# ZhangYuef/Alink

Measured on AMD Instinct MI355X. Metric: rows/sec/node + iters-to-converge, KMeans k=100 1e8-row×128-dim at 1/2/4/8 MI355X, higher is better.
Workload: dtype bf16

## Files before the change

### alink_amd/ops/_lib.py

```python
from __future__ import annotations

import ctypes
import os
from typing import Optional

import torch

__all__ = ["lib", "require", "available", "kernels_enabled", "call", "query", "LIB_PATH", "stream_ptr"]

LIB_PATH = os.environ.get("ALINK_HIP_LIB") or os.path.join(os.path.dirname(os.path.abspath(__file__)), "libalink_hip.so")
_lib: Optional[ctypes.CDLL] = None
_err: Optional[str] = None


def _load():
    global _lib, _err
    if _lib is not None or _err is not None:
        return _lib
    if not os.path.exists(LIB_PATH):
        _err = f"{LIB_PATH} not built (run python build_native.py)"
        return None
    try:
        L = ctypes.CDLL(LIB_PATH)
    except OSError as e:
# ... 19 lines not shown
    _lib = L
    return _lib


_c_i64, _c_int, _c_vp, _c_f = ctypes.c_int64, ctypes.c_int, ctypes.c_void_p, ctypes.c_float
_c_d = ctypes.c_double
_SIGNATURES = {
    "alink_kmeans_prep_centroids": [_c_vp, _c_int, _c_vp, _c_vp, _c_vp],
    "alink_kmeans_reduce_slabs": [_c_vp, _c_vp, _c_int, _c_int, _c_vp, _c_vp, _c_vp],
    "alink_tree_gather_rows": [_c_vp, _c_vp, _c_vp, _c_i64, _c_vp, _c_vp, _c_vp],
    "alink_tree_hist_fm": [_c_vp, _c_int, _c_vp, _c_vp, _c_vp, _c_int, _c_vp, _c_int, _c_int, _c_int, _c_vp, _c_int,
                           _c_int, _c_vp, _c_vp, _c_vp, _c_vp, _c_int],
    "alink_tree_hist_f32": [_c_vp, _c_i64, _c_int, _c_vp, _c_vp, _c_int, _c_int, _c_int, _c_vp, _c_int, _c_int,
                            _c_vp],
    "alink_tree_node_sums": [_c_vp, _c_vp, _c_vp, _c_i64, _c_int, _c_int, _c_vp, _c_int, _c_vp],
    "alink_tree_route": [_c_vp, _c_i64, _c_int, _c_vp, _c_vp, _c_vp, _c_vp, _c_int, _c_int, _c_vp],
    "alink_kmeans_assign_accum_bf16_v7": [_c_vp, _c_i64, _c_vp, _c_vp, _c_int, _c_vp, _c_vp, _c_int, _c_vp, _c_vp,
                                          _c_int],
    "alink_kmeans_v7_grid": [_c_i64, _c_int],
    "alink_kmeans_assign_accum_bf16_v10": [_c_vp, _c_i64, _c_vp, _c_vp, _c_int, _c_vp, _c_vp, _c_int, _c_vp, _c_vp,
                                           _c_int, _c_vp, _c_vp, _c_int, _c_d],
    "alink_kmeans_v10_grid": [_c_i64, _c_int],
    "alink_tree_predict": [_c_vp, _c_i64, _c_int, _c_int, _c_vp, _c_vp, _c_int, _c_vp, _c_vp, _c_int, _c_vp, _c_int,
                           _c_vp, _c_vp, _c_vp, _c_vp],
    "alink_tree_codes": [_c_vp, _c_int, _c_vp, _c_vp, _c_int, _c_i64, _c_i64, _c_int, _c_int, _c_vp, _c_vp],
    "alink_gbdt_rank_stats": [_c_vp, _c_vp, _c_vp, _c_vp, _c_int, _c_vp, _c_int, _c_vp, _c_vp, _c_vp, _c_vp],
    "alink_kmeans_seed_ref": [_c_vp, _c_vp, _c_vp, _c_int, _c_int, _c_int, _c_d, _c_vp, _c_vp, _c_vp, _c_vp],
    "alink_kmeans_local_lloyd": [_c_vp, _c_vp, _c_int, _c_int, _c_int, _c_vp, _c_vp, _c_vp, _c_vp, _c_vp, _c_int, _c_vp,
                                 _c_vp, _c_vp, _c_vp, _c_vp],
    "alink_kmeans_par_pick": [_c_vp, _c_i64, _c_i64, _c_i64, _c_d, _c_vp, _c_i64, _c_vp, _c_vp],
    "alink_kmeans_cost1_bf16": [_c_vp, _c_i64, _c_int, _c_vp, _c_vp, _c_vp, _c_int, _c_int, _c_vp],
    "alink_kmeans_nearest_bf16": [_c_vp, _c_i64, _c_int, _c_vp, _c_vp, _c_int, _c_int, _c_vp, _c_vp, _c_int,
                                  _c_int, _c_int, _c_vp, _c_vp],
    "alink_linear_grad_f64": [_c_vp, _c_vp, _c_vp, _c_vp, _c_i64, _c_int, _c_int, _c_d, _c_vp, _c_int, _c_vp,
                              _c_vp],
    "alink_linear_grad_pad": [_c_int],
    "alink_linear_search_f64": [_c_vp, _c_vp, _c_vp, _c_vp, _c_vp, _c_i64, _c_int, _c_int, _c_d, _c_d, _c_int, _c_vp,
                                _c_int, _c_vp, _c_vp],
    "alink_kmeans_update": [_c_vp, _c_int, _c_vp, _c_vp, _c_vp, _c_vp, _c_vp, _c_int, _c_vp, _c_d, _c_vp,
                            ctypes.c_uint64, _c_vp],
    "alink_kmeans_host_stat_alloc": [ctypes.POINTER(_c_vp), ctypes.POINTER(_c_vp)],
    "alink_kmeans_host_stat_free": [_c_vp],
    "alink_kmeans_accum_bf16": [_c_vp, _c_i64, _c_int, _c_vp, _c_vp, _c_int, _c_int, _c_vp, _c_vp, _c_vp, _c_vp],
    "alink_kmeans_accum_f32": [_c_vp, _c_i64, _c_int, _c_vp, _c_vp, _c_int, _c_int, _c_vp, _c_vp, _c_vp, _c_vp],
    "alink_kmeans_accum_kmax": [_c_int],
    "alink_kmeans_accum_mfma_bf16": [_c_vp, _c_i64, _c_vp, _c_int, _c_int, _c_vp, _c_vp, _c_vp, _c_vp],
    "alink_linear_grad_wide_f64": [_c_vp, _c_vp, _c_vp, _c_vp, _c_i64, _c_int, _c_int, _c_d, _c_vp, _c_int, _c_vp,
                                   _c_vp],
    "alink_csr_row_deriv_f64": [_c_vp, _c_vp, _c_vp, _c_vp, _c_vp, _c_vp, _c_i64, _c_int, _c_d, _c_vp, _c_vp, _c_vp],
    "alink_csc_gather_f64": [_c_vp, _c_vp, _c_vp, _c_vp, _c_i64, _c_vp, _c_vp],
    "alink_ftrl_check_indices": [_c_vp, _c_i64, _c_i64, _c_vp, _c_int, _c_vp],
    "alink_ftrl_hogwild_f64": [_c_vp, _c_vp, _c_vp, _c_vp, _c_i64, _c_vp, _c_vp, _c_vp, _c_d, _c_d, _c_d, _c_d, _c_int,
                               _c_vp],
    "alink_ftrl_partial_margin_f64": [_c_vp, _c_vp, _c_vp, _c_i64, _c_vp, _c_i64, _c_i64, _c_vp, _c_int, _c_vp],
    "alink_ftrl_coord_update_f64": [_c_vp, _c_i64, _c_vp, _c_vp, _c_vp, _c_vp, _c_vp, _c_vp, _c_i64, _c_i64, _c_d, _c_d,
                                    _c_d, _c_d, _c_i64, _c_int, _c_vp],
    "alink_ftrl_coord_scan_f64": [_c_vp, _c_vp, _c_vp, _c_i64, _c_vp, _c_vp, _c_vp, _c_vp, _c_vp, _c_i64, _c_d, _c_d,
                                  _c_d, _c_d, _c_int, _c_vp],
    "alink_ftrl_coord_long_f64": [_c_vp, _c_vp, _c_vp, _c_i64, _c_vp, _c_vp, _c_vp, _c_vp, _c_vp, _c_i64, _c_d, _c_d,
                                  _c_d, _c_d, _c_int, _c_vp],
    "alink_ftrl_prox_f64": [_c_vp, _c_i64, _c_vp, _c_vp, _c_vp, _c_d, _c_d, _c_d, _c_d, _c_int, _c_vp],
    "alink_murmur3_utf8_index": [_c_vp, _c_vp, _c_i64, _c_vp, _c_int, ctypes.c_uint32, _c_i64, _c_vp, _c_vp, _c_vp],
    "alink_murmur3_multi_index": [_c_vp, _c_int, _c_i64, ctypes.c_uint32, _c_i64, _c_vp, _c_vp, _c_vp],
    "alink_murmur3_bytes": [_c_vp, _c_vp, _c_i64, ctypes.c_uint32, _c_vp, _c_vp],
    "alink_vector_assemble": [_c_i64, _c_int, _c_vp, _c_vp, _c_vp, _c_vp, _c_int, _c_vp],
    "alink_murmur3_index": [_c_vp, _c_vp, _c_i64, _c_vp, _c_int, ctypes.c_uint32, _c_i64, _c_vp, _c_vp, _c_vp],
# ... 122 lines not shown
```

### alink_amd/ops/csrc/kmeans_v10.hip

```cpp
#include <hip/hip_runtime.h>
#include <stdint.h>
#include <stdlib.h>

#ifndef KM10_PAIRMAX
#define KM10_PAIRMAX 0
#endif

#ifndef KM10_TIMING
#define KM10_TIMING 0
#endif

#ifndef KM10_PFD
#define KM10_PFD 0
#endif

#include "kmeans_tile.h"
#include "kmeans_v10_body.h"

namespace {

using namespace kmtile;

typedef float f32x32 __attribute__((ext_vector_type(32)));
typedef float f32x16 __attribute__((ext_vector_type(16)));
typedef float f32x4v __attribute__((ext_vector_type(4)));
typedef uint32_t u32x4 __attribute__((ext_vector_type(4)));

enum Mode10 { FULL = 0, LOAD_ONLY = 1, COMPUTE_ONLY = 2, DIST_ONLY = 3, ACC_ONLY = 4 };

constexpr int NBUF = 9;
constexpr int AHEAD = 7;
constexpr int OFF_ASG = NBUF * TILE;
constexpr uint32_t IDX_MODE = 0xC000u;
constexpr int OFF_CNT = OFF_ASG + 512;
constexpr int OFF_DYN = OFF_CNT + 128 * 4;
constexpr int OFF_JUNK = OFF_DYN + 8 * 4;
constexpr int LDS_BYTES = OFF_JUNK + 256;
constexpr int CH = 16;
constexpr int RED_STRIDE = 112 * D;
static_assert(LDS_BYTES <= LDS_CAP && 2 * RED_STRIDE * 4 <= NBUF * TILE, "LDS plan");

__device__ __forceinline__ float pack(float v, uint32_t field) {
    return __uint_as_float((__float_as_uint(v) & 0xFFFFFF80u) | field);
}

__device__ __forceinline__ float max3_raw(float a, float b, float c) {
    float r;
    asm("v_max3_f32 %0, %1, %2, %3" : "=v"(r) : "v"(a), "v"(b), "v"(c));
    return r;
}
__device__ __forceinline__ float max_raw(float a, float b) {
    float r;
    asm("v_max_f32 %0, %1, %2" : "=v"(r) : "v"(a), "v"(b));
    return r;
}

template <int NT>
__device__ __forceinline__ void dma_tile(uint32_t m0v, uint32_t voff, __amdgpu_buffer_rsrc_t rs, uint32_t soff) {
    uint32_t keep, m1, s1, s2, s3;
#define KM10_DMA(POL)                                                                                       \
    asm volatile(                                                                                           \
        "s_mov_b32 %0, m0\n\t"                                                                              \
        "s_mov_b32 m0, %7\n\t"                                                                              \
        "s_add_u32 %2, %8, 4096\n\t"                                                                        \
        "buffer_load_dwordx4 %5, %6, %8 offen " POL " lds\n\t"                                              \
        "s_add_u32 %1, %7, 4096\n\t"                                                                        \
        "s_mov_b32 m0, %1\n\t"                                                                              \
        "s_add_u32 %3, %8, 8192\n\t"                                                                        \
        "buffer_load_dwordx4 %5, %6, %2 offen " POL " lds\n\t"                                              \
        "s_add_u32 %1, %7, 8192\n\t"                                                                        \
        "s_mov_b32 m0, %1\n\t"                                                                              \
        "s_add_u32 %4, %8, 12288\n\t"                                                                       \
        "buffer_load_dwordx4 %5, %6, %3 offen " POL " lds\n\t"                                              \
        "s_add_u32 %1, %7, 12288\n\t"                                                                       \
        "s_mov_b32 m0, %1\n\t"                                                                              \
        "s_nop 0\n\t"                                                                                       \
        "buffer_load_dwordx4 %5, %6, %4 offen " POL " lds\n\t"                                              \
        "s_mov_b32 m0, %0"                                                                                  \
        : "=&s"(keep), "=&s"(m1), "=&s"(s1), "=&s"(s2), "=&s"(s3)                                           \
        : "v"(voff), "s"(rs), "s"(m0v), "s"(soff)                                                           \
        : "memory")
    if constexpr (NT) KM10_DMA("nt");
    else KM10_DMA("");
#undef KM10_DMA
}

__device__ __forceinline__ void l2_touch(uint32_t m0v, uint32_t voff, __amdgpu_buffer_rsrc_t rs, uint32_t soff) {
    uint32_t keep;
    asm volatile(
        "s_mov_b32 %0, m0\n\t"
        "s_mov_b32 m0, %3\n\t"
        "s_nop 0\n\t"
        "buffer_load_dword %1, %2, %4 offen lds\n\t"
        "s_mov_b32 m0, %0"
        : "=&s"(keep)
        : "v"(voff), "s"(rs), "s"(m0v), "s"(soff)
        : "memory");
}

template <int KB, int MODE, int NT, int DYN>
__global__ __launch_bounds__(512) void kmeans_v10_kernel(const __bf16* __restrict__ Xp, int64_t N,
                                                         const __bf16* __restrict__ Cp,
                                                         const float* __restrict__ ninit, float* __restrict__ slab,
                                                         float* __restrict__ slab_cnt, int* __restrict__ assign_out,
                                                         int64_t ntiles, int64_t per, int rev,
                                                         unsigned* __restrict__ dyn_ctr, int dyn_par, int nqs,
                                                         int64_t pool_base, int npool,
                                                         const unsigned* __restrict__ skip, int pfd_arg) {
    static_assert(KB >= 1 && KB <= 7, "v10 holds at most 112 centroids in registers");
    const int pfd = KM10_PFD ? pfd_arg : 0;
    constexpr bool LOADS = MODE == FULL || MODE == LOAD_ONLY;
    __shared__ __attribute__((aligned(1024))) char lds[LDS_BYTES];
    if (skip != nullptr && __hip_atomic_load(skip, __ATOMIC_RELAXED, __HIP_MEMORY_SCOPE_AGENT) != 0u) return;
    const int tid = threadIdx.x;
    const int lane = tid & 63;
    const int wave = __builtin_amdgcn_readfirstlane(tid >> 6);
    const int g = lane >> 4;
// ... 144 lines not shown
        if (LOADS && dma_wave) {
            if (2 * j + AHEAD - 2 < ntp) stage_tile(2 * j + AHEAD - 2);
            if (2 * j + AHEAD - 1 < ntp) stage_tile(2 * j + AHEAD - 1);
        }
    };

    if (wave < 4) {
        const int myrow = 16 * wave + li;
        const int apos = 16 * ((myrow >> 2) & 3) + 4 * (myrow >> 4) + (myrow & 3);
        bf16x8 cf[KB][4];
        f32x4 nin[KB];
#pragma unroll
        for (int b = 0; b < KB; ++b) {
#pragma unroll
            for (int s = 0; s < 4; ++s)
                cf[b][s] = *reinterpret_cast<const bf16x8*>(Cp + (16 * b + li) * D + 8 * (s + 4 * g));
            nin[b] = *reinterpret_cast<const f32x4*>(ninit + 16 * b + 4 * g);
        }
        int xr[4];
#pragma unroll
        for (int s = 0; s < 4; ++s) xr[s] = xoff(myrow, s + 4 * g);
        auto load_frag = [&](uint32_t slot, bf16x8 (&x)[4]) {
            const char* xt = lds + slot;
#pragma unroll
            for (int s = 0; s < 4; ++s) x[s] = *reinterpret_cast<const bf16x8*>(xt + xr[s]);
        };
        auto cross_max = [&](float run) {
            const uint32_t u = __float_as_uint(run);
            const auto p32 = __builtin_amdgcn_permlane32_swap(u, u, false, false);
            const uint32_t u2 = __float_as_uint(max_raw(__uint_as_float(p32[0]), __uint_as_float(p32[1])));
            const auto p16 = __builtin_amdgcn_permlane16_swap(u2, u2, false, false);
            return __float_as_uint(max_raw(__uint_as_float(p16[0]), __uint_as_float(p16[1])));
        };
        auto rare_neg = [&](const bf16x8 (&x)[4], uint32_t u, uint32_t c) {
            float run = -3.4e38f;
#pragma unroll
            for (int b = 0; b < KB; ++b) {
                f32x4 acc = nin[b];
#pragma unroll
                for (int s = 0; s < 4; ++s) acc = __builtin_amdgcn_mfma_f32_16x16x32_bf16(cf[b][s], x[s], acc, 0, 0, 0);
                const uint32_t c0 = (uint32_t)(16 * b + 4 * g);
                run = max3_raw(run, pack(acc[0], c0), pack(acc[1], c0 + 1));
                run = max3_raw(run, pack(acc[2], c0 + 2), pack(acc[3], c0 + 3));
            }
            const uint32_t v = cross_max(run);
            return (int32_t)u < 0 ? (v & 127u) : c;
        };
        auto tile_max = [&](const bf16x8 (&x)[4]) {
            f32x4 acc[KB];
            float run = -3.4e38f;
#pragma unroll
            for (int b = 0; b <= KB + 1; ++b) {
                if (b < KB) {
                    acc[b] = nin[b];
#pragma unroll
                    for (int s = 0; s < 4; ++s)
                        acc[b] = __builtin_amdgcn_mfma_f32_16x16x32_bf16(cf[b][s], x[s], acc[b], 0, 0, 0);
                }
                if (b >= 2) {
                    const uint32_t f0 = 127u - (uint32_t)(16 * (b - 2) + 4 * g);
                    run = max3_raw(run, pack(acc[b - 2][0], f0), pack(acc[b - 2][1], f0 - 1));
                    run = max3_raw(run, pack(acc[b - 2][2], f0 - 2), pack(acc[b - 2][3], f0 - 3));
                }
                if (b < KB && b >= 2) {
#pragma unroll
                    for (int s = 0; s < 3; ++s) {
                        __builtin_amdgcn_sched_group_barrier(0x008, 1, 0);
                        __builtin_amdgcn_sched_group_barrier(0x002, 2, 0);
                    }
                    __builtin_amdgcn_sched_group_barrier(0x008, 1, 0);
                }
                __builtin_amdgcn_sched_barrier(0);
            }
            const uint32_t u = cross_max(run);
            uint32_t c = 127u - (u & 127u);
            if (__builtin_amdgcn_ballot_w64((int32_t)u < 0) != 0) c = rare_neg(x, u, c);
            return c;
        };
        auto pair_max = [&](const bf16x8 (&xa_)[4], const bf16x8 (&xb_)[4], uint32_t& ca, uint32_t& cb) {
            f32x4 aA[KB], aB[KB];
            float runA = -3.4e38f, runB = -3.4e38f;
#pragma unroll
            for (int b = 0; b <= KB + 1; ++b) {
                if (b < KB) {
                    aA[b] = nin[b];
                    aB[b] = nin[b];
#pragma unroll
                    for (int s = 0; s < 4; ++s) {
                        aA[b] = __builtin_amdgcn_mfma_f32_16x16x32_bf16(cf[b][s], xa_[s], aA[b], 0, 0, 0);
                        aB[b] = __builtin_amdgcn_mfma_f32_16x16x32_bf16(cf[b][s], xb_[s], aB[b], 0, 0, 0);
                    }
                }
                if (b >= 2) {
                    const uint32_t f0 = 127u - (uint32_t)(16 * (b - 2) + 4 * g);
                    runA = max3_raw(runA, pack(aA[b - 2][0], f0), pack(aA[b - 2][1], f0 - 1));
                    runA = max3_raw(runA, pack(aA[b - 2][2], f0 - 2), pack(aA[b - 2][3], f0 - 3));
                    runB = max3_raw(runB, pack(aB[b - 2][0], f0), pack(aB[b - 2][1], f0 - 1));
                    runB = max3_raw(runB, pack(aB[b - 2][2], f0 - 2), pack(aB[b - 2][3], f0 - 3));
                }
                if (b < KB && b >= 2) {
#pragma unroll
                    for (int s = 0; s < 6; ++s) {
                        __builtin_amdgcn_sched_group_barrier(0x008, 1, 0);
                        __builtin_amdgcn_sched_group_barrier(0x002, 2, 0);
                    }
                    __builtin_amdgcn_sched_group_barrier(0x008, 2, 0);
                }
                __builtin_amdgcn_sched_barrier(0);
            }
            const uint32_t uA = cross_max(runA), uB = cross_max(runB);
            ca = 127u - (uA & 127u);
            cb = 127u - (uB & 127u);
            if (__builtin_amdgcn_ballot_w64((int32_t)(uA | uB) < 0) != 0) {
                ca = rare_neg(xa_, uA, ca);
                cb = rare_neg(xb_, uB, cb);
            }
        };
        const int64_t row_end = DYN ? N : ((tbase + nt) * TR < N ? (tbase + nt) * TR : N);
        auto publish = [&](int j, int h, uint32_t c) {
            if (g == 0) {
                const int64_t grow = (DYN ? dphys(2 * j + h) : tbase + phys(2 * j + h)) * TR + myrow;
                reinterpret_cast<uint16_t*>(lds + OFF_ASG)[(j & 1) * 128 + h * 64 + apos] =
                    (uint16_t)(IDX_MODE | (2 * c));
                if (grow < row_end) {
                    __hip_atomic_fetch_add(cnt + c, 1u, __ATOMIC_RELAXED, __HIP_MEMORY_SCOPE_WORKGROUP);
                    if (assign_out != nullptr) assign_out[grow] = (int)c;
                }
            }
        };
        bf16x8 xa[4], xb[4];
        int pend = 0;
        unsigned pend_v = 0u;
        uint32_t slot_a = 0;
#if KM10_TIMING
        const uint64_t loop0 = __builtin_readcyclecounter();
#endif
        for (int j = 0; DYN || j <= np; ++j) {
            pre(j);
            if constexpr (DYN) {
                if (j > np_dyn) break;
                if (wave == 0) {
                    int nq = dstate[2 * (j & 1)], done = dstate[2 * (j & 1) + 1];
                    if (pend) {
                        const unsigned r = __builtin_amdgcn_readfirstlane(pend_v);
                        if ((int)r < npool) {
                            if (lane == 0)
                                qbase[nq & 3] = (int)(pool_base + (int64_t)(rev ? npool - 1 - (int)r : (int)r) * CH);
                            ++nq;
                        } else {
                            done = 1;
                        }
                        pend = 0;
                    }
                    if (!done && nq <= (2 * j + 2 * AHEAD - 4) / CH) {
                        if (lane == 0)
                            pend_v = __hip_atomic_fetch_add(dyn_ctr + dyn_par, 1u, __ATOMIC_RELAXED,
                                                            __HIP_MEMORY_SCOPE_AGENT);
                        pend = 1;
                    }
                    if (lane == 0) {
                        dstate[2 * ((j + 1) & 1)] = nq;
                        dstate[2 * ((j + 1) & 1) + 1] = done;
                    }
                }
            }
            const int npj = DYN ? np_dyn : np;
            if (MODE == LOAD_ONLY || MODE == ACC_ONLY || j >= npj) continue;
            const uint32_t slot_b = next_slot(slot_a);
            load_frag(slot_a, xa);
            load_frag(slot_b, xb);
            slot_a = next_slot(slot_b);
            uint32_t c0, c1;
            if constexpr (KM10_PAIRMAX) {
                pair_max(xa, xb, c0, c1);
            } else {
                c0 = tile_max(xa);
                c1 = tile_max(xb);
            }
            publish(j, 0, c0);
            publish(j, 1, c1);
#if KM10_TIMING
            if (j == 0 && tid == 0) stamp[1] = (int64_t)__builtin_amdgcn_s_memrealtime();
#endif
        }
#if KM10_TIMING
        if (tid == 0) {
            stamp[2] = (int64_t)__builtin_amdgcn_s_memrealtime();
            stamp[8] = (int64_t)wait_vm_cyc;
            stamp[9] = (int64_t)wait_bar_cyc;
            stamp[10] = (int64_t)(__builtin_readcyclecounter() - loop0);
        }
#endif
        barrier_lds();
        barrier_lds();
        barrier_lds();
    } else {
        const int a = wave - 4;
        const uint32_t aoff =
            lbase + (uint32_t)(a * 1024) + ((uint32_t)(16 * (lane >> 2) + 4 * (lane & 3)) ^ (uint32_t)(a << 4));
        f32x32 s0 = {}, s1 = {}, s2 = {}, s3 = {}, s4 = {}, s5 = {}, s6 = {};
        f32x16 xv = {};
        auto acc_tile = [&](uint32_t slot, const u32x4& v0, const u32x4& v1) {
            const uint32_t w0 = __builtin_amdgcn_readfirstlane(v0[0]), w1 = __builtin_amdgcn_readfirstlane(v0[1]);
            const uint32_t w2 = __builtin_amdgcn_readfirstlane(v0[2]), w3 = __builtin_amdgcn_readfirstlane(v0[3]);
            const uint32_t w4 = __builtin_amdgcn_readfirstlane(v1[0]), w5 = __builtin_amdgcn_readfirstlane(v1[1]);
            const uint32_t w6 = __builtin_amdgcn_readfirstlane(v1[2]), w7 = __builtin_amdgcn_readfirstlane(v1[3]);
            const uint32_t base = aoff + slot;
            f32x4v addr;
            uint32_t keep;
            asm volatile(KM10_ACC_BODY
                         : "+{v[32:63]}"(s0), "+{v[64:95]}"(s1), "+{v[96:127]}"(s2), "+{v[128:159]}"(s3),
// ... 190 lines not shown
```

### alink_amd/ops/kmeans.py

```python
from __future__ import annotations

import os
import weakref
from typing import Dict, Optional, Tuple

import numpy as np
import torch

from . import _lib
from . import kmeans_dense64 as _d64

__all__ = ["assign_accumulate", "assign", "assign_accumulate_torch", "hip_supported", "prepare_centroids",
           "general_supported", "assign_accumulate_general_hip", "accumulate_by_index_hip", "f32_supported",
           "assign_accumulate_f32_hip", "assign_f32"]

_BUF: Dict[Tuple, Tuple[torch.Tensor, torch.Tensor]] = {}
HIP_CALLS = 0
HIP_D = 128
HIP_KMAX = 128


def hip_supported(X: torch.Tensor, k: int) -> bool:
    return (X.is_cuda and X.dtype == torch.bfloat16 and X.dim() == 2 and X.shape[1] == HIP_D
            and 1 <= k <= HIP_KMAX and X.shape[0] > 0 and X.is_contiguous() and X.data_ptr() % 16 == 0)
# ... 297 lines not shown

def cost1_hip(X: torch.Tensor, c: torch.Tensor, with_sum: bool = False):
    if not nearest_supported(X):
        raise ValueError("cost1_hip needs contiguous bf16 [N, D] on GPU with D in (64, 128, 256)")
    n, d = X.shape
    cb = c.reshape(-1).to(device=X.device, dtype=torch.bfloat16).contiguous()
    if cb.numel() != d:
        raise ValueError("center shape mismatch")
    cost = torch.empty(n, dtype=torch.float64, device=X.device)
    grid = COST1_GRID * _num_cus(X.device)
    wsum = torch.empty(grid * 4, dtype=torch.float64, device=X.device) if with_sum else None
    _lib.call("alink_kmeans_cost1_bf16", X.data_ptr(), n, d, cb.data_ptr(), cost.data_ptr(),
              None if wsum is None else wsum.data_ptr(), grid, COST1_VARIANT, _lib.stream_ptr(X.device))
    return (cost, wsum) if with_sum else cost


def nearest_counts_hip(X: torch.Tensor, C: torch.Tensor) -> torch.Tensor:
    if not nearest_supported(X):
        raise ValueError("nearest_counts_hip needs contiguous bf16 [N, D] on GPU with D in (64, 128, 256)")
    n, d = X.shape
    m = C.shape[0]
    if m > NEAREST_CHUNK:
        return torch.bincount(nearest_hip(X, C)[0].to(torch.int64), minlength=m)
    Cb = C.to(device=X.device, dtype=torch.bfloat16).contiguous()
    if Cb.shape[1] != d or m == 0:
        raise ValueError("centroid shape mismatch")
    chalf = (0.5 * (Cb.float() ** 2).sum(1)).contiguous()
    counts = torch.zeros(m, dtype=torch.int64, device=X.device)
    _lib.call("alink_kmeans_nearest_bf16", X.data_ptr(), n, d, Cb.data_ptr(), chalf.data_ptr(), m, 0, None, None, 0,
              NEAREST_GRID * _num_cus(X.device), _rg(d, m), counts.data_ptr(), _lib.stream_ptr(X.device))
    return counts


def _scores(Xc: torch.Tensor, C: torch.Tensor, emulate_bf16: bool) -> torch.Tensor:
    if emulate_bf16:
        cb = C.to(torch.bfloat16).float()
        return Xc.float() @ cb.T - 0.5 * (cb ** 2).sum(1)
    Cd = C.to(Xc.dtype)
    return Xc @ Cd.T - 0.5 * (Cd ** 2).sum(1)


def assign_accumulate_torch(X: torch.Tensor, C: torch.Tensor, weights: Optional[torch.Tensor] = None,
                            chunk: int = 1 << 20) -> torch.Tensor:
    k, d = C.shape
    out = torch.zeros((k, d + 1), dtype=torch.float64, device=X.device)
    low = X.dtype in (torch.bfloat16, torch.float16)
    for s in range(0, X.shape[0], chunk):
        xc = X[s:s + chunk]
        if not low:
            xc = xc.to(torch.float64)
        idx = _scores(xc, C, low).argmax(1)
        w = None if weights is None else weights[s:s + chunk].to(torch.float64)
        xs = xc.to(torch.float64)
        if w is not None:
            xs = xs * w[:, None]
        out[:, :d].index_add_(0, idx, xs)
        out[:, d].index_add_(0, idx, torch.ones_like(idx, dtype=torch.float64) if w is None else w)
    return out


def general_supported(X: torch.Tensor, k: int) -> bool:
    return nearest_supported(X) and 1 <= k <= (512 if X.shape[1] == 64 else 256)


GENERAL_CALLS = 0
_ACC: Dict[Tuple, Tuple[torch.Tensor, torch.Tensor]] = {}
# ... 271 lines not shown
```

### alink_amd/ops/kmeans_rows.py

```python
from __future__ import annotations

from typing import Optional

import torch

from . import _lib, bisecting as bops, kmeans as kops, kmeans_dense64 as kd64, kmeans_sparse as ksp
from .kmeans_sparse import sparse_selected

__all__ = ["rows", "Rows", "column_kind", "sparse_selected", "sparse_rows", "pairwise_distance"]

CHUNK = 1 << 20
SPARSE_CHUNK = 1 << 16
SPARSE, DENSE, UNDECIDED = 1, 0, -1


def pairwise_distance(X: torch.Tensor, C: torch.Tensor, distance_type: str) -> torch.Tensor:
    dt = distance_type.upper()
    if dt == "COSINE":
        return 1.0 - X @ C.T
    if dt == "HAVERSINE":
        lat1 = torch.deg2rad(X[:, 0:1])
        lon1 = torch.deg2rad(X[:, 1:2])
        lat2 = torch.deg2rad(C[:, 0])[None, :]
        lon2 = torch.deg2rad(C[:, 1])[None, :]
# ... 189 lines not shown
    def _descend(self, table, slot, levels, grid):
        return _torch_descend(lambda M: self.X @ M.T, table, slot, levels)

    def _child_stats(self, slot, nslots, sqnorm, grid, work=None):
        from .gemm import tn_matmul
        X, d = self.X, self.d
        ok = (slot >= 0) & (slot < nslots)
        Xs, ps = X[ok], slot[ok].to(torch.int64)
        norm2 = self.row_sqnorm()[ok]
        onehot = torch.nn.functional.one_hot(ps, nslots).to(X.dtype)
        return torch.zeros((nslots, d + 2), dtype=torch.float64, device=X.device) + tn_matmul(
            onehot, torch.cat([Xs, torch.ones_like(norm2)[:, None], norm2[:, None]], 1))

    def queue_assign(self, k):
        if not kops.hip_supported(self.X, k):
            return None
        return lambda C, step, skip: kops.assign_accumulate_hip(self.X, C, reverse=kops.serpentine_reverse(step),
                                                                skip=skip)


class _Bf16Rows(_TorchRows):

    def nearest(self, C, dist_all=None):
        if C.shape[0] == 1:
            return torch.zeros(1, dtype=torch.int64, device=self.device).expand(self.n), kops.cost1_hip(self.X, C[0])
        idx, d2 = kops.nearest_hip(self.X, C)
        return idx.to(torch.int64), d2.to(torch.float64).sqrt_()

    def first_cost(self, c):
        cost, psum = kops.cost1_hip(self.X, c[0], with_sum=True)
        return cost, psum.sum()

    def nearest_counts(self, C):
        return kops.nearest_counts_hip(self.X, C)


class _Dense64Rows(_TorchRows):

    def nearest(self, C, dist_all=None):
        if dist_all is not None:
            return super().nearest(C, dist_all)
        idx, d2 = kd64.nearest(self.X, C, self.dist_type)
        return idx, (d2.sqrt_() if self.dist_type == "EUCLIDEAN" else d2)

    def nearest_counts(self, C):
        return kd64.nearest_counts(self.X, C, self.dist_type)

    def _descend(self, table, slot, levels, grid):
        if kd64.use_hip(self.X, 1):
            return bops.descend_f64(self.X, table, slot, levels, grid)
        return super()._descend(table, slot, levels, grid)

    def _child_stats(self, slot, nslots, sqnorm, grid, work=None):
        if not kd64.use_hip(self.X, nslots):
            return super()._child_stats(slot, nslots, sqnorm, grid)
        X, d = self.X, self.d
        if work is None:
            work = kd64.sorted_work(slot, nslots, ignore_outside=True)
        buf = torch.zeros((nslots, d + 2), dtype=torch.float64, device=X.device)
        buf[:, :d + 1] = kd64.accumulate_work(X, work, nslots, grid)
        if sqnorm:
            buf[:, d + 1] = kd64.accumulate_work(self.row_sqnorm()[:, None], work, nslots, grid)[:, 0]
        return buf


def rows(X, dist_type: str) -> Rows:
# ... 15 lines not shown
```

Measured before the change: 23.54 billion.

## Add ring-buffered MFMA kernel for k-means candidate weight counting

Adds a dedicated HIP kernel that counts nearest-candidate assignments for up to 224 bf16 candidates of 128 dims. It reuses the v10 LDS ring-DMA staging (shared helpers are moved into a header) and splits the candidate blocks across two wave groups, merging partial argmax results through LDS. Counts are accumulated with LDS atomics per workgroup. The bf16 rows path now uses this kernel for nearest_counts when the input is large enough. This is meant to replace the generic nearest kernel in the k-means|| weighting step. It adds a second specialized kernel to maintain, and the two-half merge is new logic whose tie-breaking may differ slightly from the old path.

```diff
diff --git a/alink_amd/ops/_lib.py b/alink_amd/ops/_lib.py
--- a/alink_amd/ops/_lib.py
+++ b/alink_amd/ops/_lib.py
@@ -75,6 +75,7 @@
     "alink_kmeans_cost1_bf16": [_c_vp, _c_i64, _c_int, _c_vp, _c_vp, _c_vp, _c_int, _c_int, _c_vp],
     "alink_kmeans_nearest_bf16": [_c_vp, _c_i64, _c_int, _c_vp, _c_vp, _c_int, _c_int, _c_vp, _c_vp, _c_int,
                                   _c_int, _c_int, _c_vp, _c_vp],
+    "alink_kmeans_weights_bf16_ring": [_c_vp, _c_i64, _c_vp, _c_int, _c_vp, _c_int, _c_int, _c_vp],
     "alink_linear_grad_f64": [_c_vp, _c_vp, _c_vp, _c_vp, _c_i64, _c_int, _c_int, _c_d, _c_vp, _c_int, _c_vp,
                               _c_vp],
     "alink_linear_grad_pad": [_c_int],
diff --git a/alink_amd/ops/csrc/kmeans_ring.h b/alink_amd/ops/csrc/kmeans_ring.h
--- /dev/null
+++ b/alink_amd/ops/csrc/kmeans_ring.h
@@ -0,0 +1,66 @@
+#pragma once
+#include "kmeans_tile.h"
+
+namespace kmring {
+
+using namespace kmtile;
+
+constexpr int NBUF = 9;
+constexpr int AHEAD = 7;
+
+__device__ __forceinline__ float max3_raw(float a, float b, float c) {
+    float r;
+    asm("v_max3_f32 %0, %1, %2, %3" : "=v"(r) : "v"(a), "v"(b), "v"(c));
+    return r;
+}
+__device__ __forceinline__ float max_raw(float a, float b) {
+    float r;
+    asm("v_max_f32 %0, %1, %2" : "=v"(r) : "v"(a), "v"(b));
+    return r;
+}
+
+template <int NT>
+__device__ __forceinline__ void dma_tile(uint32_t m0v, uint32_t voff, __amdgpu_buffer_rsrc_t rs, uint32_t soff) {
+    uint32_t keep, m1, s1, s2, s3;
+#define KM10_DMA(POL)                                                                                       \
+    asm volatile(                                                                                           \
+        "s_mov_b32 %0, m0\n\t"                                                                              \
+        "s_mov_b32 m0, %7\n\t"                                                                              \
+        "s_add_u32 %2, %8, 4096\n\t"                                                                        \
+        "buffer_load_dwordx4 %5, %6, %8 offen " POL " lds\n\t"                                              \
+        "s_add_u32 %1, %7, 4096\n\t"                                                                        \
+        "s_mov_b32 m0, %1\n\t"                                                                              \
+        "s_add_u32 %3, %8, 8192\n\t"                                                                        \
+        "buffer_load_dwordx4 %5, %6, %2 offen " POL " lds\n\t"                                              \
+        "s_add_u32 %1, %7, 8192\n\t"                                                                        \
+        "s_mov_b32 m0, %1\n\t"                                                                              \
+        "s_add_u32 %4, %8, 12288\n\t"                                                                       \
+        "buffer_load_dwordx4 %5, %6, %3 offen " POL " lds\n\t"                                              \
+        "s_add_u32 %1, %7, 12288\n\t"                                                                       \
+        "s_mov_b32 m0, %1\n\t"                                                                              \
+        "s_nop 0\n\t"                                                                                       \
+        "buffer_load_dwordx4 %5, %6, %4 offen " POL " lds\n\t"                                              \
+        "s_mov_b32 m0, %0"                                                                                  \
+        : "=&s"(keep), "=&s"(m1), "=&s"(s1), "=&s"(s2), "=&s"(s3)                                           \
+        : "v"(voff), "s"(rs), "s"(m0v), "s"(soff)                                                           \
+        : "memory")
+    if constexpr (NT) KM10_DMA("nt");
+    else KM10_DMA("");
+#undef KM10_DMA
+}
+
+__device__ __forceinline__ uint32_t ring_next_slot(uint32_t s) {
+    return s == (uint32_t)((NBUF - 1) * TILE) ? 0u : s + (uint32_t)TILE;
+}
+
+__device__ __forceinline__ uint32_t ring_lane_offset(int tid) {
+    const int prow = (tid & 255) >> 4;
+    return (uint32_t)(prow * ROWB + ((tid & 15) ^ xsw(prow)) * 16);
+}
+
+__device__ __forceinline__ void ring_wait_pair(int j, int ntp) {
+    const int issued = 2 * j + AHEAD - 3 < ntp - 1 ? 2 * j + AHEAD - 3 : ntp - 1;
+    wait_tile_np<4, 3>(issued - (2 * j + 1));
+}
+
+}
diff --git a/alink_amd/ops/csrc/kmeans_v10.hip b/alink_amd/ops/csrc/kmeans_v10.hip
--- a/alink_amd/ops/csrc/kmeans_v10.hip
+++ b/alink_amd/ops/csrc/kmeans_v10.hip
@@ -15,11 +15,13 @@
 #endif
 
 #include "kmeans_tile.h"
+#include "kmeans_ring.h"
 #include "kmeans_v10_body.h"
 
 namespace {
 
 using namespace kmtile;
+using namespace kmring;
 
 typedef float f32x32 __attribute__((ext_vector_type(32)));
 typedef float f32x16 __attribute__((ext_vector_type(16)));
@@ -28,8 +30,6 @@
 
 enum Mode10 { FULL = 0, LOAD_ONLY = 1, COMPUTE_ONLY = 2, DIST_ONLY = 3, ACC_ONLY = 4 };
 
-constexpr int NBUF = 9;
-constexpr int AHEAD = 7;
 constexpr int OFF_ASG = NBUF * TILE;
 constexpr uint32_t IDX_MODE = 0xC000u;
 constexpr int OFF_CNT = OFF_ASG + 512;
@@ -42,47 +42,6 @@
 
 __device__ __forceinline__ float pack(float v, uint32_t field) {
     return __uint_as_float((__float_as_uint(v) & 0xFFFFFF80u) | field);
-}
-
-__device__ __forceinline__ float max3_raw(float a, float b, float c) {
-    float r;
-    asm("v_max3_f32 %0, %1, %2, %3" : "=v"(r) : "v"(a), "v"(b), "v"(c));
-    return r;
-}
-__device__ __forceinline__ float max_raw(float a, float b) {
-    float r;
-    asm("v_max_f32 %0, %1, %2" : "=v"(r) : "v"(a), "v"(b));
-    return r;
-}
-
-template <int NT>
-__device__ __forceinline__ void dma_tile(uint32_t m0v, uint32_t voff, __amdgpu_buffer_rsrc_t rs, uint32_t soff) {
-    uint32_t keep, m1, s1, s2, s3;
-#define KM10_DMA(POL)                                                                                       \
-    asm volatile(                                                                                           \
-        "s_mov_b32 %0, m0\n\t"                                                                              \
-        "s_mov_b32 m0, %7\n\t"                                                                              \
-        "s_add_u32 %2, %8, 4096\n\t"                                                                        \
-        "buffer_load_dwordx4 %5, %6, %8 offen " POL " lds\n\t"                                              \
-        "s_add_u32 %1, %7, 4096\n\t"                                                                        \
-        "s_mov_b32 m0, %1\n\t"                                                                              \
-        "s_add_u32 %3, %8, 8192\n\t"                                                                        \
-        "buffer_load_dwordx4 %5, %6, %2 offen " POL " lds\n\t"                                              \
-        "s_add_u32 %1, %7, 8192\n\t"                                                                        \
-        "s_mov_b32 m0, %1\n\t"                                                                              \
-        "s_add_u32 %4, %8, 12288\n\t"                                                                       \
-        "buffer_load_dwordx4 %5, %6, %3 offen " POL " lds\n\t"                                              \
-        "s_add_u32 %1, %7, 12288\n\t"                                                                       \
-        "s_mov_b32 m0, %1\n\t"                                                                              \
-        "s_nop 0\n\t"                                                                                       \
-        "buffer_load_dwordx4 %5, %6, %4 offen " POL " lds\n\t"                                              \
-        "s_mov_b32 m0, %0"                                                                                  \
-        : "=&s"(keep), "=&s"(m1), "=&s"(s1), "=&s"(s2), "=&s"(s3)                                           \
-        : "v"(voff), "s"(rs), "s"(m0v), "s"(soff)                                                           \
-        : "memory")
-    if constexpr (NT) KM10_DMA("nt");
-    else KM10_DMA("");
-#undef KM10_DMA
 }
 
 __device__ __forceinline__ void l2_touch(uint32_t m0v, uint32_t voff, __amdgpu_buffer_rsrc_t rs, uint32_t soff) {
diff --git a/alink_amd/ops/csrc/kmeans_weights.hip b/alink_amd/ops/csrc/kmeans_weights.hip
--- /dev/null
+++ b/alink_amd/ops/csrc/kmeans_weights.hip
@@ -0,0 +1,299 @@
+#include <hip/hip_runtime.h>
+#include <stdint.h>
+
+#include "kmeans_tile.h"
+#include "kmeans_ring.h"
+
+namespace {
+
+using namespace kmtile;
+using namespace kmring;
+
+constexpr int MMAX = 224;
+constexpr int IMG_BIAS = MMAX * D * 2;
+constexpr int OFF_RES = NBUF * TILE;
+constexpr int OFF_CNT = OFF_RES + 2 * 2 * TR * 8;
+constexpr int LDS_BYTES = OFF_CNT + MMAX * 4;
+constexpr float kNone = -3.4e38f;
+constexpr uint32_t kNoIdx = 0x7fffffffu;
+static_assert(LDS_BYTES <= LDS_CAP, "LDS plan");
+
+template <int N>
+struct Int {
+    static constexpr int value = N;
+};
+
+template <int N, int I = 0, class F>
+__device__ __forceinline__ void static_for(F&& f) {
+    if constexpr (I < N) {
+        f(Int<I>{});
+        static_for<N, I + 1>(f);
+    }
+}
+
+__device__ __forceinline__ float cross_max(float run) {
+    const uint32_t u = __float_as_uint(run);
+    const auto p32 = __builtin_amdgcn_permlane32_swap(u, u, false, false);
+    const uint32_t u2 = __float_as_uint(max_raw(__uint_as_float(p32[0]), __uint_as_float(p32[1])));
+    const auto p16 = __builtin_amdgcn_permlane16_swap(u2, u2, false, false);
+    return max_raw(__uint_as_float(p16[0]), __uint_as_float(p16[1]));
+}
+__device__ __forceinline__ uint32_t cross_min(uint32_t u) {
+    const auto p32 = __builtin_amdgcn_permlane32_swap(u, u, false, false);
+    const uint32_t u2 = p32[0] < p32[1] ? p32[0] : p32[1];
+    const auto p16 = __builtin_amdgcn_permlane16_swap(u2, u2, false, false);
+    return p16[0] < p16[1] ? p16[0] : p16[1];
+}
+
+template <int KB, int H0, int NT>
+__global__ __launch_bounds__(512) void kmeans_weights_kernel(const __bf16* __restrict__ Xp, int64_t N,
+                                                             const char* __restrict__ img, int m,
+                                                             unsigned long long* __restrict__ counts,
+                                                             int64_t ntiles, int64_t per) {
+    static_assert(KB >= 1 && KB <= 14 && H0 >= 1 && H0 <= 7 && KB - H0 >= 0 && KB - H0 <= 7, "7 blocks per half");
+    __shared__ __attribute__((aligned(1024))) char lds[LDS_BYTES];
+    const int tid = threadIdx.x;
+    const int lane = tid & 63;
+    const int wave = __builtin_amdgcn_readfirstlane(tid >> 6);
+    const int g = lane >> 4;
+    const int li = lane & 15;
+    const int64_t tbase = (int64_t)blockIdx.x * per;
+    const int nt = (int)(ntiles > tbase ? (ntiles - tbase < per ? ntiles - tbase : per) : 0);
+    const int np = (nt + 1) >> 1;
+    const int ntp = 2 * np;
+    const uint32_t lbase = (uint32_t)(uintptr_t)(LDS_AS void*)lds;
+    uint32_t* const cnt = reinterpret_cast<uint32_t*>(lds + OFF_CNT);
+    float* const res = reinterpret_cast<float*>(lds + OFF_RES);
+    const __bf16* const Cp = reinterpret_cast<const __bf16*>(img);
+    const float* const bias = reinterpret_cast<const float*>(img + IMG_BIAS);
+    const int64_t row_end = (tbase + nt) * TR < N ? (tbase + nt) * TR : N;
+    const int myrow = 16 * (wave & 3) + li;
+
+    const uint32_t voff = ring_lane_offset(tid);
+    const int64_t rem_rows = N - tbase * TR;
+    const int64_t region = rem_rows * ROWB < (int64_t)nt * TILE ? rem_rows * ROWB : (int64_t)nt * TILE;
+    const __amdgpu_buffer_rsrc_t rs = __builtin_amdgcn_make_buffer_rsrc(
+        (void*)(reinterpret_cast<const char*>(Xp) + tbase * TILE), (short)0, (int)(region > 0 ? region : 0),
+        0x00020000);
+    const uint32_t m0_wave = lbase + (uint32_t)((wave - 4) * 1024);
+    uint32_t stage_slot = 0, stage_off = 0;
+    auto stage_next = [&]() {
+        dma_tile<NT>(__builtin_amdgcn_readfirstlane(m0_wave + stage_slot), voff, rs,
+                     __builtin_amdgcn_readfirstlane(stage_off));
+        stage_slot = ring_next_slot(stage_slot);
+        stage_off += (uint32_t)TILE;
+    };
+    auto pre = [&](int j, auto loader_c) {
+        constexpr bool LOADER = decltype(loader_c)::value != 0;
+        if (LOADER && j < np) ring_wait_pair(j, ntp);
+        barrier_lds();
+        if (LOADER) {
+            if (2 * j + AHEAD - 2 < ntp) stage_next();
+            if (2 * j + AHEAD - 1 < ntp) stage_next();
+        }
+    };
+
+    auto role = [&](auto nbh_c, auto b0_c, auto upper_c) {
+        constexpr int NBH = decltype(nbh_c)::value;
+        constexpr int B0 = decltype(b0_c)::value;
+        constexpr bool UPPER = decltype(upper_c)::value != 0;
+        constexpr int NBR = NBH > 0 ? NBH : 1;
+        constexpr bool MERGE = KB - H0 > 0;
+        bf16x8 cf[NBR][4];
+        f32x4 nin[NBR];
+        if constexpr (NBH > 0) {
+#pragma unroll
+            for (int b = 0; b < NBH; ++b) {
+#pragma unroll
+                for (int s = 0; s < 4; ++s)
+                    cf[b][s] = *reinterpret_cast<const bf16x8*>(Cp + (16 * (B0 + b) + li) * D + 8 * (s + 4 * g));
+                nin[b] = *reinterpret_cast<const f32x4*>(bias + 16 * (B0 + b) + 4 * g);
+            }
+#pragma unroll
+            for (int b = 0; b < NBH; ++b)
+                asm volatile("" : "+v"(cf[b][0]), "+v"(cf[b][1]), "+v"(cf[b][2]), "+v"(cf[b][3]), "+v"(nin[b]));
+        }
+        if (UPPER) {
+            for (int s = 0; s < AHEAD - 2; ++s)
+                if (s < ntp) stage_next();
+        }
+        int xr[4];
+#pragma unroll
+        for (int s = 0; s < 4; ++s) xr[s] = xoff(myrow, s + 4 * g);
+        auto load_x = [&](uint32_t slot, bf16x8 (&x)[4]) {
+            const char* xt = lds + slot;
+#pragma unroll
+            for (int s = 0; s < 4; ++s) x[s] = *reinterpret_cast<const bf16x8*>(xt + xr[s]);
+        };
+        auto mf4 = [](f32x4& acc, const bf16x8 (&a)[4], const bf16x8 (&x)[4], const f32x4& init) {
+            asm volatile("v_mfma_f32_16x16x32_bf16 %0, %1, %2, %3" : "=&v"(acc) : "v"(a[0]), "v"(x[0]), "v"(init));
+            asm volatile("v_mfma_f32_16x16x32_bf16 %0, %1, %2, %0" : "+v"(acc) : "v"(a[1]), "v"(x[1]));
+            asm volatile("v_mfma_f32_16x16x32_bf16 %0, %1, %2, %0" : "+v"(acc) : "v"(a[2]), "v"(x[2]));
+            asm volatile("v_mfma_f32_16x16x32_bf16 %0, %1, %2, %0" : "+v"(acc) : "v"(a[3]), "v"(x[3]));
+        };
+        auto mx = [](float& run, const f32x4& acc) {
+            asm volatile("v_max3_f32 %0, %0, %1, %2" : "+v"(run) : "v"(acc[0]), "v"(acc[1]));
+            asm volatile("v_max3_f32 %0, %0, %1, %2" : "+v"(run) : "v"(acc[2]), "v"(acc[3]));
+        };
+        auto settle = [](f32x4& acc) { asm volatile("s_nop 15\n\ts_nop 7" : "+v"(acc)); };
+        auto sw = [](uint32_t& jl, const f32x4& acc, float best, auto g_c) {
+            constexpr int G = decltype(g_c)::value;
+            uint64_t m3, m2, m1, m0;
+            asm volatile(
+                "v_cmp_eq_f32 %1, %5, %9\n\t"
+                "v_cmp_eq_f32 %2, %6, %9\n\t"
+                "v_cmp_eq_f32 %3, %7, %9\n\t"
+                "v_cmp_eq_f32 %4, %8, %9\n\t"
+                "v_cndmask_b32 %0, %0, %10, %1\n\t"
+                "v_cndmask_b32 %0, %0, %11, %2\n\t"
+                "v_cndmask_b32 %0, %0, %12, %3\n\t"
+                "v_cndmask_b32 %0, %0, %13, %4"
+                : "+v"(jl), "=&s"(m3), "=&s"(m2), "=&s"(m1), "=&s"(m0)
+                : "v"(acc[3]), "v"(acc[2]), "v"(acc[1]), "v"(acc[0]), "v"(best), "n"(4 * G + 3), "n"(4 * G + 2),
+                  "n"(4 * G + 1), "n"(4 * G));
+        };
+        auto fin = [&](uint32_t jl) {
+            const uint32_t c = jl == kNoIdx ? kNoIdx : (uint32_t)(16 * B0 + 4 * g) + 16u * (jl >> 2) + (jl & 3u);
+            return cross_min(c);
+        };
+        constexpr int LATE = NBH < 2 ? NBH : 2;
+        auto pair_best = [&](uint32_t slot_a, uint32_t slot_b, float& bA, uint32_t& cA, float& bB, uint32_t& cB) {
+            bf16x8 xa[4], xb[4];
+            load_x(slot_a, xa);
+            load_x(slot_b, xb);
+            f32x4 aA[NBR], aB[NBR];
+            float runA = kNone, runB = kNone;
+            uint32_t jA = kNoIdx, jB = kNoIdx;
+            static_for<NBH>([&](auto bc) {
+                constexpr int b = decltype(bc)::value;
+                mf4(aA[b], cf[b], xa, nin[b]);
+                if constexpr (b >= 2) mx(runA, aA[b - 2]);
+            });
+            static_for<NBH>([&](auto bc) {
+                constexpr int b = decltype(bc)::value;
+                mf4(aB[b], cf[b], xb, nin[b]);
+                if constexpr (b == 1) {
+                    static_for<LATE>([&](auto tc) { mx(runA, aA[NBH - LATE + decltype(tc)::value]); });
+                    bA = cross_max(runA);
+                }
+                if constexpr (b >= 2) {
+                    sw(jA, aA[NBH + 1 - b], bA, Int<NBH + 1 - b>{});
+                    mx(runB, aB[b - 2]);
+                }
+            });
+            settle(aB[NBR - 1]);
+            if constexpr (NBH == 1) {
+                mx(runA, aA[0]);
+                bA = cross_max(runA);
+            }
+            static_for<LATE>([&](auto tc) { sw(jA, aA[LATE - 1 - decltype(tc)::value], bA, Int<LATE - 1 - decltype(tc)::value>{}); });
+            cA = fin(jA);
+            static_for<LATE>([&](auto tc) { mx(runB, aB[NBH - LATE + decltype(tc)::value]); });
+            bB = cross_max(runB);
+            static_for<NBH>([&](auto tc) { sw(jB, aB[NBH - 1 - decltype(tc)::value], bB, Int<NBH - 1 - decltype(tc)::value>{}); });
+            cB = fin(jB);
+        };
+        float pb0 = kNone, pb1 = kNone;
+        uint32_t pi0 = kNoIdx, pi1 = kNoIdx;
+        uint32_t slot_a = 0;
+        auto count_row = [&](int jp, int t, float b, uint32_t c) {
+            if constexpr (MERGE) {
+                const float* r = res + (((jp & 1) * 2 + t) * TR + myrow) * 2;
+                const float ub = r[0];
+                const uint32_t uc = __float_as_uint(r[1]);
+                if (ub > b) {
+                    b = ub;
+                    c = uc;
+                }
+            }
+            const int64_t grow = (tbase + 2 * jp + t) * TR + myrow;
+            if (grow < row_end && b > kNone && c < (uint32_t)m)
+                __hip_atomic_fetch_add(cnt + c, 1u, __ATOMIC_RELAXED, __HIP_MEMORY_SCOPE_WORKGROUP);
+        };
+        for (int j = 0; j <= np; ++j) {
+            pre(j, Int<UPPER>{});
+            if (!UPPER && j > 0 && g == 0) {
+                count_row(j - 1, 0, pb0, pi0);
+                count_row(j - 1, 1, pb1, pi1);
+            }
+            if (j >= np) continue;
+            if constexpr (NBH > 0) {
+                const uint32_t slot_b = ring_next_slot(slot_a);
+                float b0, b1;
+                uint32_t c0, c1;
+                pair_best(slot_a, slot_b, b0, c0, b1, c1);
+                slot_a = ring_next_slot(slot_b);
+                if constexpr (!UPPER) {
+                    pb0 = b0; pi0 = c0;
+                    pb1 = b1; pi1 = c1;
+                } else {
+                    if (g == 0) {
+                        float* r = res + (((j & 1) * 2) * TR + myrow) * 2;
+                        r[0] = b0;
+                        r[1] = __uint_as_float(c0);
+                        r[2 * TR] = b1;
+                        r[2 * TR + 1] = __uint_as_float(c1);
+                    }
+                }
+            }
+        }
+    };
+
+    if (tid < MMAX) cnt[tid] = 0u;
+    if (wave < 4) role(Int<H0>{}, Int<0>{}, Int<0>{});
+    else role(Int<KB - H0>{}, Int<H0>{}, Int<1>{});
+    barrier_lds();
+    if (tid < m && cnt[tid] != 0u) atomicAdd(counts + tid, (unsigned long long)cnt[tid]);
+}
+
+template <int KB, int NT>
+hipError_t launch_w(dim3 grid, hipStream_t st, const __bf16* X, int64_t N, const char* img, int m,
+                    unsigned long long* counts, int64_t ntiles, int64_t per) {
+    hipLaunchKernelGGL((kmeans_weights_kernel<KB, (KB + 1) / 2, NT>), grid, dim3(512), 0, st, X, N, img, m, counts,
+                       ntiles, per);
+    return hipGetLastError();
+}
+
+template <int NT>
+hipError_t launch_kb(int KB, dim3 grid, hipStream_t st, const __bf16* X, int64_t N, const char* img, int m,
+                     unsigned long long* counts, int64_t ntiles, int64_t per) {
+    switch (KB) {
+        case 1: return launch_w<1, NT>(grid, st, X, N, img, m, counts, ntiles, per);
+        case 2: return launch_w<2, NT>(grid, st, X, N, img, m, counts, ntiles, per);
+        case 3: return launch_w<3, NT>(grid, st, X, N, img, m, counts, ntiles, per);
+        case 4: return launch_w<4, NT>(grid, st, X, N, img, m, counts, ntiles, per);
+        case 5: return launch_w<5, NT>(grid, st, X, N, img, m, counts, ntiles, per);
+        case 6: return launch_w<6, NT>(grid, st, X, N, img, m, counts, ntiles, per);
+        case 7: return launch_w<7, NT>(grid, st, X, N, img, m, counts, ntiles, per);
+        case 8: return launch_w<8, NT>(grid, st, X, N, img, m, counts, ntiles, per);
+        case 9: return launch_w<9, NT>(grid, st, X, N, img, m, counts, ntiles, per);
+        case 10: return launch_w<10, NT>(grid, st, X, N, img, m, counts, ntiles, per);
+        case 11: return launch_w<11, NT>(grid, st, X, N, img, m, counts, ntiles, per);
+        case 12: return launch_w<12, NT>(grid, st, X, N, img, m, counts, ntiles, per);
+        case 13: return launch_w<13, NT>(grid, st, X, N, img, m, counts, ntiles, per);
+        default: return launch_w<14, NT>(grid, st, X, N, img, m, counts, ntiles, per);
+    }
+}
+
+}
+
+extern "C" {
+
+int alink_kmeans_weights_bf16_ring(const void* X, int64_t N, const void* img, int m, void* counts, int grid,
+                                   int flags, void* stream) {
+    if (N <= 0 || m < 1 || m > MMAX || grid <= 0 || ((uintptr_t)X & 15) != 0 || ((uintptr_t)img & 15) != 0) return -1;
+    const int KB = (m + 15) / 16;
+    const int64_t ntiles = (N + TR - 1) / TR;
+    if (grid > ntiles) grid = (int)ntiles;
+    const int64_t per = (ntiles + grid - 1) / grid;
+    if (per * TILE >= ((int64_t)1 << 31)) return -1;
+    hipStream_t st = reinterpret_cast<hipStream_t>(stream);
+    const __bf16* Xb = reinterpret_cast<const __bf16*>(X);
+    const char* ib = reinterpret_cast<const char*>(img);
+    unsigned long long* cp = reinterpret_cast<unsigned long long*>(counts);
+    const hipError_t e = (flags & 1) ? launch_kb<1>(KB, dim3(grid), st, Xb, N, ib, m, cp, ntiles, per)
+                                     : launch_kb<0>(KB, dim3(grid), st, Xb, N, ib, m, cp, ntiles, per);
+    return (int)e;
+}
+
+}
diff --git a/alink_amd/ops/kmeans.py b/alink_amd/ops/kmeans.py
--- a/alink_amd/ops/kmeans.py
+++ b/alink_amd/ops/kmeans.py
@@ -353,6 +353,45 @@
     return counts
 
 
+WEIGHTS_RING_D = 128
+WEIGHTS_RING_MMAX = 224
+WEIGHTS_RING_FLAGS = int(os.environ.get("ALINK_KMEANS_WEIGHTS_RING_FLAGS", "0"))
+WEIGHTS_RING_CALLS = 0
+WEIGHTS_RING_MIN_TILES = 512
+
+
+def weights_ring_selected(X: torch.Tensor, m: int) -> bool:
+    return (os.environ.get("ALINK_KMEANS_WEIGHTS_RING", "1") != "0" and nearest_supported(X)
+            and X.shape[1] == WEIGHTS_RING_D and 1 <= m <= WEIGHTS_RING_MMAX
+            and X.shape[0] >= WEIGHTS_RING_MIN_TILES * 64 * _num_cus(X.device))
+
+
+def weights_image(C: torch.Tensor, device=None) -> torch.Tensor:
+    m = C.shape[0]
+    if not 1 <= m <= WEIGHTS_RING_MMAX or C.shape[1] != WEIGHTS_RING_D:
+        raise ValueError("weights_image needs 1..224 candidates of 128 dims")
+    Cb = C.to(device=device if device is not None else C.device, dtype=torch.bfloat16).contiguous()
+    cpad = torch.zeros((WEIGHTS_RING_MMAX, WEIGHTS_RING_D), dtype=torch.bfloat16, device=Cb.device)
+    cpad[:m] = Cb
+    bias = torch.full((WEIGHTS_RING_MMAX,), -3.0e38, dtype=torch.float32, device=Cb.device)
+    bias[:m] = -(0.5 * (Cb.float() ** 2).sum(1))
+    return torch.cat([cpad.view(torch.uint8).reshape(-1), bias.view(torch.uint8)])
+
+
+def nearest_counts_ring_hip(X: torch.Tensor, C: torch.Tensor, grid: Optional[int] = None) -> torch.Tensor:
+    global WEIGHTS_RING_CALLS
+    m = C.shape[0]
+    if not (nearest_supported(X) and X.shape[1] == WEIGHTS_RING_D and 1 <= m <= WEIGHTS_RING_MMAX):
+        raise ValueError("nearest_counts_ring_hip needs contiguous 16-byte aligned bf16 [N, 128] on GPU and "
+                         "1 <= m <= 224")
+    img = weights_image(C, X.device)
+    counts = torch.zeros(m, dtype=torch.int64, device=X.device)
+    WEIGHTS_RING_CALLS += 1
+    _lib.call("alink_kmeans_weights_bf16_ring", X.data_ptr(), X.shape[0], img.data_ptr(), m, counts.data_ptr(),
+              int(grid) if grid is not None else _num_cus(X.device), WEIGHTS_RING_FLAGS, _lib.stream_ptr(X.device))
+    return counts
+
+
 def _scores(Xc: torch.Tensor, C: torch.Tensor, emulate_bf16: bool) -> torch.Tensor:
     if emulate_bf16:
         cb = C.to(torch.bfloat16).float()
diff --git a/alink_amd/ops/kmeans_rows.py b/alink_amd/ops/kmeans_rows.py
--- a/alink_amd/ops/kmeans_rows.py
+++ b/alink_amd/ops/kmeans_rows.py
@@ -245,6 +245,8 @@
         return cost, psum.sum()
 
     def nearest_counts(self, C):
+        if kops.weights_ring_selected(self.X, C.shape[0]):
+            return kops.nearest_counts_ring_hip(self.X, C)
         return kops.nearest_counts_hip(self.X, C)
 
 
```

Result: no change. 23.58 billion (median of 2 runs) (+0.2%).

## Interleave both tiles' MFMA chains with argmax packing and overlap cross-lane reduction

Applied to the files above, without the earlier changes.

Replaces the two sequential per-tile argmax passes with a single fused loop that runs tile A's then tile B's MFMA blocks back-to-back. The pack/max3 work for block t-2 is interleaved between individual MFMAs with explicit sched barriers, and tile A's permlane cross-lane reduction is spread into the MFMA slots of tile B. It also moves the per-lane group offset out of the per-element pack field into one add/subtract after the running max, and keeps the mask in a VGPR. The aim is to hide VALU and permlane latency behind matrix-core work. The cost is register pressure from 2*KB accumulators, plus correctness now depends on the carry-free field arithmetic.

```diff
diff --git a/alink_amd/ops/csrc/kmeans_v10.hip b/alink_amd/ops/csrc/kmeans_v10.hip
--- a/alink_amd/ops/csrc/kmeans_v10.hip
+++ b/alink_amd/ops/csrc/kmeans_v10.hip
@@ -1,10 +1,6 @@
 #include <hip/hip_runtime.h>
 #include <stdint.h>
 #include <stdlib.h>
-
-#ifndef KM10_PAIRMAX
-#define KM10_PAIRMAX 0
-#endif
 
 #ifndef KM10_TIMING
 #define KM10_TIMING 0
@@ -40,9 +36,6 @@
 constexpr int RED_STRIDE = 112 * D;
 static_assert(LDS_BYTES <= LDS_CAP && 2 * RED_STRIDE * 4 <= NBUF * TILE, "LDS plan");
 
-__device__ __forceinline__ float pack(float v, uint32_t field) {
-    return __uint_as_float((__float_as_uint(v) & 0xFFFFFF80u) | field);
-}
 
 __device__ __forceinline__ float max3_raw(float a, float b, float c) {
     float r;
@@ -293,6 +286,10 @@
             const auto p16 = __builtin_amdgcn_permlane16_swap(u2, u2, false, false);
             return __float_as_uint(max_raw(__uint_as_float(p16[0]), __uint_as_float(p16[1])));
         };
+        uint32_t keepmask;
+        asm volatile("v_mov_b32 %0, 0xffffff80" : "=v"(keepmask));
+        const uint32_t g4 = 4u * (uint32_t)g;
+        auto packs = [&](float v, uint32_t field) { return __uint_as_float((__float_as_uint(v) & keepmask) | field); };
         auto rare_neg = [&](const bf16x8 (&x)[4], uint32_t u, uint32_t c) {
             float run = -3.4e38f;
 #pragma unroll
@@ -300,76 +297,70 @@
                 f32x4 acc = nin[b];
 #pragma unroll
                 for (int s = 0; s < 4; ++s) acc = __builtin_amdgcn_mfma_f32_16x16x32_bf16(cf[b][s], x[s], acc, 0, 0, 0);
-                const uint32_t c0 = (uint32_t)(16 * b + 4 * g);
-                run = max3_raw(run, pack(acc[0], c0), pack(acc[1], c0 + 1));
-                run = max3_raw(run, pack(acc[2], c0 + 2), pack(acc[3], c0 + 3));
-            }
-            const uint32_t v = cross_max(run);
+                const uint32_t c0 = (uint32_t)(16 * b);
+                run = max3_raw(run, packs(acc[0], c0), packs(acc[1], c0 + 1));
+                run = max3_raw(run, packs(acc[2], c0 + 2), packs(acc[3], c0 + 3));
+            }
+            const uint32_t v = cross_max(__uint_as_float(__float_as_uint(run) + g4));
             return (int32_t)u < 0 ? (v & 127u) : c;
         };
-        auto tile_max = [&](const bf16x8 (&x)[4]) {
-            f32x4 acc[KB];
-            float run = -3.4e38f;
-#pragma unroll
-            for (int b = 0; b <= KB + 1; ++b) {
-                if (b < KB) {
-                    acc[b] = nin[b];
-#pragma unroll
-                    for (int s = 0; s < 4; ++s)
-                        acc[b] = __builtin_amdgcn_mfma_f32_16x16x32_bf16(cf[b][s], x[s], acc[b], 0, 0, 0);
-                }
-                if (b >= 2) {
-                    const uint32_t f0 = 127u - (uint32_t)(16 * (b - 2) + 4 * g);
-                    run = max3_raw(run, pack(acc[b - 2][0], f0), pack(acc[b - 2][1], f0 - 1));
-                    run = max3_raw(run, pack(acc[b - 2][2], f0 - 2), pack(acc[b - 2][3], f0 - 3));
-                }
-                if (b < KB && b >= 2) {
-#pragma unroll
-                    for (int s = 0; s < 3; ++s) {
-                        __builtin_amdgcn_sched_group_barrier(0x008, 1, 0);
-                        __builtin_amdgcn_sched_group_barrier(0x002, 2, 0);
-                    }
-                    __builtin_amdgcn_sched_group_barrier(0x008, 1, 0);
+        auto pair_max = [&](const bf16x8 (&xa_)[4], const bf16x8 (&xb_)[4], uint32_t& ca, uint32_t& cb) {
+            f32x4 acc[2 * KB];
+            float run[2] = {-3.4e38f, -3.4e38f};
+            float p0 = 0.f, p1 = 0.f, p2 = 0.f, p3 = 0.f;
+            uint32_t uA = 0u, w0 = 0u, w1 = 0u;
+            auto seam = [&](int i) {
+                if (i == 0) {
+                    uA = __float_as_uint(run[0]) - g4;
+                    const auto p32 = __builtin_amdgcn_permlane32_swap(uA, uA, false, false);
+                    w0 = p32[0];
+                    w1 = p32[1];
+                } else if (i == 1) {
+                    const uint32_t u2 = __float_as_uint(max_raw(__uint_as_float(w0), __uint_as_float(w1)));
+                    const auto p16 = __builtin_amdgcn_permlane16_swap(u2, u2, false, false);
+                    w0 = p16[0];
+                    w1 = p16[1];
+                } else {
+                    uA = __float_as_uint(max_raw(__uint_as_float(w0), __uint_as_float(w1)));
+                }
+            };
+#pragma unroll
+            for (int t = 0; t < 2 * KB + 2; ++t) {
+                const bool mf = t < 2 * KB, vl = t >= 2;
+                const int b = t < KB ? t : t - KB;
+                const int pt = (t - 2) / KB, pb = (t - 2) % KB;
+                const uint32_t f0 = 127u - (uint32_t)(16 * pb);
+                auto mfma = [&](int s) {
+                    if (!mf) return;
+                    acc[t] = __builtin_amdgcn_mfma_f32_16x16x32_bf16(cf[b][s], t < KB ? xa_[s] : xb_[s],
+                                                                     s == 0 ? nin[b] : acc[t], 0, 0, 0);
+                };
+                mfma(0);
+                if (vl) {
+                    p0 = packs(acc[t - 2][0], f0);
+                    p1 = packs(acc[t - 2][1], f0 - 1);
                 }
                 __builtin_amdgcn_sched_barrier(0);
-            }
-            const uint32_t u = cross_max(run);
-            uint32_t c = 127u - (u & 127u);
-            if (__builtin_amdgcn_ballot_w64((int32_t)u < 0) != 0) c = rare_neg(x, u, c);
-            return c;
-        };
-        auto pair_max = [&](const bf16x8 (&xa_)[4], const bf16x8 (&xb_)[4], uint32_t& ca, uint32_t& cb) {
-            f32x4 aA[KB], aB[KB];
-            float runA = -3.4e38f, runB = -3.4e38f;
-#pragma unroll
-            for (int b = 0; b <= KB + 1; ++b) {
-                if (b < KB) {
-                    aA[b] = nin[b];
-                    aB[b] = nin[b];
-#pragma unroll
-                    for (int s = 0; s < 4; ++s) {
-                        aA[b] = __builtin_amdgcn_mfma_f32_16x16x32_bf16(cf[b][s], xa_[s], aA[b], 0, 0, 0);
-                        aB[b] = __builtin_amdgcn_mfma_f32_16x16x32_bf16(cf[b][s], xb_[s], aB[b], 0, 0, 0);
-                    }
-                }
-                if (b >= 2) {
-                    const uint32_t f0 = 127u - (uint32_t)(16 * (b - 2) + 4 * g);
-                    runA = max3_raw(runA, pack(aA[b - 2][0], f0), pack(aA[b - 2][1], f0 - 1));
-                    runA = max3_raw(runA, pack(aA[b - 2][2], f0 - 2), pack(aA[b - 2][3], f0 - 3));
-                    runB = max3_raw(runB, pack(aB[b - 2][0], f0), pack(aB[b - 2][1], f0 - 1));
-                    runB = max3_raw(runB, pack(aB[b - 2][2], f0 - 2), pack(aB[b - 2][3], f0 - 3));
-                }
-                if (b < KB && b >= 2) {
-#pragma unroll
-                    for (int s = 0; s < 6; ++s) {
-                        __builtin_amdgcn_sched_group_barrier(0x008, 1, 0);
-                        __builtin_amdgcn_sched_group_barrier(0x002, 2, 0);
-                    }
-                    __builtin_amdgcn_sched_group_barrier(0x008, 2, 0);
+                mfma(1);
+                if (vl) {
+                    run[pt] = max3_raw(run[pt], p0, p1);
+                    p2 = packs(acc[t - 2][2], f0 - 2);
                 }
                 __builtin_amdgcn_sched_barrier(0);
-            }
-            const uint32_t uA = cross_max(runA), uB = cross_max(runB);
+                mfma(2);
+                if (vl) {
+                    p3 = packs(acc[t - 2][3], f0 - 3);
+                    run[pt] = max3_raw(run[pt], p2, p3);
+                }
+                __builtin_amdgcn_sched_barrier(0);
+                mfma(3);
+                if (mf && t >= KB + 2 && t < KB + 5) seam(t - KB - 2);
+                __builtin_amdgcn_sched_barrier(0);
+            }
+#pragma unroll
+            for (int i = 0; i < 3; ++i)
+                if (KB + 2 + i >= 2 * KB) seam(i);
+            const uint32_t uB = cross_max(__uint_as_float(__float_as_uint(run[1]) - g4));
             ca = 127u - (uA & 127u);
             cb = 127u - (uB & 127u);
             if (__builtin_amdgcn_ballot_w64((int32_t)(uA | uB) < 0) != 0) {
@@ -432,12 +423,7 @@
             load_frag(slot_b, xb);
             slot_a = next_slot(slot_b);
             uint32_t c0, c1;
-            if constexpr (KM10_PAIRMAX) {
-                pair_max(xa, xb, c0, c1);
-            } else {
-                c0 = tile_max(xa);
-                c1 = tile_max(xb);
-            }
+            pair_max(xa, xb, c0, c1);
             publish(j, 0, c0);
             publish(j, 1, c1);
 #if KM10_TIMING
```

Measured after the change: 23.80 billion before, 24.06 billion after (median of 6 runs). 1.01x the previous value.
